# yjpark1/multiagent_rl

Measured on AMD Instinct MI355X. Metric: env-steps/sec, simple_spread N=6 x B envs, 1/2/4/8 MI355X, higher is better.
Workload: dtype f32

## Files before the change

### multiagent_rl_amd/csrc/pw_kernels_spread_quad.hpp

```cpp
#pragma once

#include "pw_kernels_spread.hpp"

namespace {

__device__ __forceinline__ void quad_pair_of(const int q, int &i, int &j)
{
    i = q < 5 ? 0 : q < 9 ? 1 : q < 12 ? 2 : q < 14 ? 3 : 4;
    j = q - (i == 0 ? 0 : i == 1 ? 5 : i == 2 ? 9 : i == 3 ? 12 : 14) + i + 1;
}

__device__ __forceinline__ void quad_act_fetch(const int32_t *row, const uint32_t lane_off, const uint32_t lds_slot, const uint32_t slot_read)
{
    unsigned keep;
    asm volatile("s_mov_b32 %0, m0\n\ts_mov_b32 m0, %3\n\ts_nop 0\n\tglobal_load_lds_dword %1, %2\n\ts_mov_b32 m0, %0"
                 : "=&s"(keep) : "v"(lane_off), "s"(row), "s"(lds_slot), "v"(slot_read) : "memory");
}

template <bool K1>
__device__ __forceinline__ void quad_pair_force(const float2 qi, const float2 qj, const uint32_t near_lo, const uint32_t near_span,
                                                const float dist_min, const float k, const float cf, float &Fx, float &Fy)
{
    const float dx = qi.x - qj.x, dy = qi.y - qj.y;
    const float d2 = dx * dx + dy * dy;
    const f32x2 a = {cf * dx, cf * dy};
    const bool near = __float_as_uint(d2) - near_lo >= near_span;
    const bool uni = (k >= 9.094947017729282e-13f) & (k <= 1099511627776.0f) & (cf >= 9.5367431640625e-07f) & (cf <= 128.0f);
    const bool c1 = (__float_as_uint(d2) - 0x12800000u) < (0x6C800000u - 0x12800000u);
    const bool c2 = fminf(fabsf(a.x), fabsf(a.y)) >= 8.673617379884035e-19f;
    const bool fast = near & c1 & c2 & uni;
    const bool any_cold = __builtin_amdgcn_ballot_w64(near & !fast) != 0;
    Fx = 0.0f; Fy = 0.0f;
    if (fast) {
        const float dist = sqrt_rn_core(d2);
        const float y0 = __builtin_amdgcn_rcpf(dist);
        __builtin_amdgcn_sched_barrier(0);
        const float yd = __builtin_fmaf(__builtin_fmaf(-dist, y0, 1.0f), y0, y0);
        const f32x2 Q = div_chain2(a, dist, yd);
        const float xarg = K1 ? div_chain1(-(dist - dist_min), k, div_refined_rcp(k))
                              : div_chain(-(dist - dist_min), k, div_refined_rcp(k));
        const float pen = softplus_branchless(xarg) * k;
        const f32x2 F = Q * f32x2{pen, pen};
        Fx = F.x;
        Fy = F.y;
    }
    if (__builtin_expect(any_cold, 0)) {
        if (near & !fast) collision_force_pair<true, K1>(qi.x, qi.y, qj.x, qj.y, dist_min, k, cf, Fx, Fy);
    }
}

template <bool COLL>
__device__ __forceinline__ void quad_coll_tests(const float2 mine, const float2 (&q6)[6], const float coll_thr2, int &cnt, uint32_t &cmask)
{
    cnt = 0; cmask = 0;
#if defined(PW_EXPERIMENTS) && defined(PW_EXP_NO_COLL_TESTS)
    cnt = 1;
#else
#pragma unroll
    for (int j = 0; j < 6; ++j) {
        const float2 q = q6[j];
        const float dx = q.x - mine.x, dy = q.y - mine.y;
        const float d2 = dx * dx + dy * dy;
        cnt += d2 < coll_thr2 ? 1 : 0;
        if (COLL) cmask |= d2 < coll_thr2 ? 1u << j : 0u;
    }
#endif
}

#ifndef PW_QUAD_BARRIER
#define PW_QUAD_BARRIER(t) duo_barrier()
#endif
#ifndef PW_QUAD_ACT_AHEAD
#define PW_QUAD_ACT_AHEAD 4
#endif
#ifndef PW_QUAD_PAD_P
#define PW_QUAD_PAD_P()
#endif
#ifndef PW_QUAD_PAD_OB
#define PW_QUAD_PAD_OB()
#endif
constexpr int kQuadActAhead = PW_QUAD_ACT_AHEAD;
constexpr int kQuadN = 6, kQuadL = 6, kQuadEPP = 4, kQuadEPW = 8;
struct SpreadQuadLds { float4 *s_ring; float2 *s_ftab, *s_lmB, *s_utab; float *s_min, *s_rew; int32_t *s_act; uint32_t bytes; };
__host__ __device__ inline SpreadQuadLds spread_quad_lds(unsigned char *raw = nullptr)
{
    LdsCursor c{reinterpret_cast<float *>(raw)}; SpreadQuadLds o;
    o.s_ring = c.take<float4>(4 * kWave);
    o.s_ftab = c.take<float2>(2 * kQuadEPP * kQuadN * kQuadN);
    o.s_min = c.take<float>(kWave); o.s_rew = c.take<float>(kWave);
    o.s_lmB = c.take<float2>(kQuadEPW * kQuadL); o.s_act = c.take<int32_t>(2 * kQuadActAhead * kWave);
    o.s_utab = c.take<float2>(2 * 8);
    o.bytes = 4 * c.at; return o;
}
template <bool UNIT_MASS, bool COLL = false, bool K1 = false>
__global__ void __launch_bounds__(4 * kWave) pw_spread_quad_kernel(const StreamParams A, const int T)
{
    constexpr int N = kQuadN, L = kQuadL, D = 16, P2 = 15, EPP = kQuadEPP, EPW = kQuadEPW;
    extern __shared__ __attribute__((aligned(16))) unsigned char smem_raw[];
    const SpreadQuadLds Y = spread_quad_lds(smem_raw);

    const int wave = __builtin_amdgcn_readfirstlane((((int)threadIdx.x >> 6) + 2 * (((int)blockIdx.x >> 8) & 1)) & 3);
    const int lane = (int)threadIdx.x & 63;
    const int env0 = (int)blockIdx.x * EPW;
    const int envs_here = A.B - env0 < EPW ? A.B - env0 : EPW;
    const size_t BN = (size_t)A.B * N;

    const bool resets = A.auto_reset && A.max_episode_len > 0;
    int offs_all = A.ep_step[env0 + (lane < envs_here ? lane : 0)];
    auto next_reset_step = [&](int t_from) -> int {
        if (!resets) return 0x7fffffff;
        int rem = A.max_episode_len - 1 - (t_from + offs_all);
        rem = rem < 0 ? 0 : rem;
        int m = 0x7fffffff;
        for (int e = 0; e < envs_here; ++e) {
            const int r = __builtin_amdgcn_readlane(rem, e);
            m = r < m ? r : m;
        }
        return t_from + m;
    };
    int t_reset = next_reset_step(0);
    auto reset_step_update = [&](int t) {
        if (t + 1 + offs_all >= A.max_episode_len) offs_all = -(t + 1);
        t_reset = next_reset_step(t + 1);
    };
    int cur = 0;

    if (wave < 2) {
        __builtin_amdgcn_s_setprio(3);
        const int e0 = wave * EPP;
        const int nv = envs_here - e0 < 0 ? 0 : envs_here - e0 < EPP ? envs_here - e0 : EPP;
        if (nv == 0) {
            for (int t = 0; t < T; ++t) PW_QUAD_BARRIER(t);
            return;
        }
        const int la = lane < nv * N ? lane : 0;
        const int e4 = la / N, a = la - e4 * N;
        const int me = (e0 + e4) * N + a;
        const int env = env0 + e0 + e4;
        const uint32_t g = (uint32_t)env * (uint32_t)N + (uint32_t)a;
        const uint64_t env_id = A.env_id_base + (uint64_t)env;
        const int lp = lane < nv * P2 ? lane : 0;
        const int pe = lp / P2, pq = lp - pe * P2;
        int pi, pj;
        quad_pair_of(pq, pi, pj);
        const int ri = (e0 + pe) * N + pi, rj = (e0 + pe) * N + pj;
        float2 *ftab = Y.s_ftab + wave * (EPP * N * N);
        float2 *f_ij = ftab + (pe * N + pi) * N + (pj - 1), *f_ji = ftab + (pe * N + pj) * N + pi;
        const float2 *row = ftab + (e4 * N + a) * N;

        float px = A.pos_x[g], py = A.pos_y[g], vx = A.vel_x[g], vy = A.vel_y[g];
        int ep_off = A.ep_step[env];
        uint32_t ep_count = A.ep_count[env];
        Y.s_ring[me] = make_float4(px, py, vx, vy);
        float2 *utab = Y.s_utab + wave * 8;
        if (lane < 6) {
            const int ai = lane;
            float ux = 0.0f + ((ai == 1 ? 1.0f : 0.0f) - (ai == 2 ? 1.0f : 0.0f));
            float uy = 0.0f + ((ai == 3 ? 1.0f : 0.0f) - (ai == 4 ? 1.0f : 0.0f));
            ux *= A.sens; uy *= A.sens;
            if (A.fscale != 1.0f) { ux = A.fscale * ux; uy = A.fscale * uy; }
            utab[lane] = make_float2(ux + 0.0f, uy + 0.0f);
        }
        wave_lds_sync();
        const float k = A.contact_margin, cf = A.contact_force, dt = A.dt, damp = A.damp, mass = A.mass;
        const uint32_t near_lo = __float_as_uint(A.near_thr2), near_span = 0x7F800000u - near_lo;
        const unsigned char *act_row = reinterpret_cast<const unsigned char *>(A.act);
        const size_t act_stride = BN * sizeof(int32_t);
        const uint32_t act_off = g * (uint32_t)sizeof(int32_t);
        int32_t *act_ring = Y.s_act + wave * (kQuadActAhead * kWave);
        const uint32_t act_lds = __builtin_amdgcn_readfirstlane((uint32_t)reinterpret_cast<uintptr_t>(act_ring));
        auto fetch_act = [&](int t, uint32_t slot_read) {
            quad_act_fetch(reinterpret_cast<const int32_t *>(act_row), act_off, act_lds + (uint32_t)(t & (kQuadActAhead - 1)) * (kWave * 4), slot_read);
            act_row += t + 1 < T ? act_stride : (size_t)0;
        };
        asm volatile("" :: "v"(ep_off), "v"(ep_count), "v"(offs_all), "v"(px), "v"(py), "v"(vx), "v"(vy), "s"(t_reset));
        for (int t0 = 0; t0 < kQuadActAhead; ++t0) fetch_act(t0, 0u);
        float2 qi = *reinterpret_cast<const float2 *>(Y.s_ring + ri);
        float2 qj = *reinterpret_cast<const float2 *>(Y.s_ring + rj);
        PW_STAMP_DECL;
        for (int t = 0; t < T; ++t) {
            PW_STAMP_START;
            asm volatile("s_waitcnt vmcnt(%0)" :: "n"(kQuadActAhead - 1) : "memory");
            PW_STAMP(3);
            const uint32_t ai = (uint32_t)act_ring[(t & (kQuadActAhead - 1)) * kWave + lane];
            fetch_act(t + kQuadActAhead, ai);
            const float2 u0 = utab[ai < 5u ? ai : 5u];
            const bool two_slots = t == t_reset;
            float Fx, Fy;
            quad_pair_force<K1>(qi, qj, near_lo, near_span, A.dist_min, k, cf, Fx, Fy);
            *f_ij = make_float2(Fx, Fy);
            *f_ji = make_float2(-Fx, -Fy);
            PW_STAMP(0);
            float fx = u0.x, fy = u0.y;
            asm volatile("" ::: "memory");
#pragma unroll
            for (int j = 0; j < N - 1; ++j) {
                const float2 F = row[j];
                fx = F.x + fx;
                fy = F.y + fy;
            }
            vx = vx * damp; vy = vy * damp;
            vx = vx + div_mass<UNIT_MASS>(fx, mass) * dt;
            vy = vy + div_mass<UNIT_MASS>(fy, mass) * dt;
            px = px + vx * dt;
            py = py + vy * dt;
            int nxt = (cur + 1) & 3;
            Y.s_ring[nxt * kWave + me] = make_float4(px, py, vx, vy);
            if (__builtin_expect(two_slots, 0)) {
                if (t + 1 + ep_off >= A.max_episode_len) {
                    ep_count += 1;
                    ep_off = -(t + 1);
                    pw_reset_xy(A.seed, env_id, ep_count, (uint32_t)a, -1.0f, 1.0f, &px, &py);
                    vx = 0.f; vy = 0.f;
                }
                reset_step_update(t);
                nxt = (nxt + 1) & 3;
                Y.s_ring[nxt * kWave + me] = make_float4(px, py, vx, vy);
            }
            cur = nxt;
            asm volatile("" ::: "memory");
            qi = *reinterpret_cast<const float2 *>(Y.s_ring + cur * kWave + ri);
            qj = *reinterpret_cast<const float2 *>(Y.s_ring + cur * kWave + rj);
            PW_STAMP(1);
            PW_QUAD_PAD_P();
            PW_QUAD_BARRIER(t);
            PW_STAMP(2);
        }
        act_fetch_drain();
#ifdef PW_STAMPS
        if (blockIdx.x == 0 && wave == 0 && lane == 0)
            for (int i_ = 0; i_ < 4; ++i_) g_pw_stamps[i_] = st_acc[i_];
#endif
        A.pos_x[g] = px; A.pos_y[g] = py;
        A.vel_x[g] = vx; A.vel_y[g] = vy;
        A.ep_step[env] = T + ep_off;
        A.ep_count[env] = ep_count;
        return;
    }

    int e_local = lane / N;
    int a = lane - e_local * N;
    if (e_local >= envs_here) { e_local = 0; a = 0; }
    const int env = env0 + e_local;
    const int base = e_local * N, me = base + a;
    const uint32_t g = (uint32_t)env * (uint32_t)N + (uint32_t)a;
    const uint64_t env_id = A.env_id_base + (uint64_t)env;
    int ep_off = A.ep_step[env];
    uint32_t ep_count = A.ep_count[env];
    float olx = A.lm_x[(size_t)env * L + a], oly = A.lm_y[(size_t)env * L + a];

    if (wave == 2) {
        float own_p = 0.0f;
        int cnt_p = 0;
        const int *cnt_w = reinterpret_cast<const int *>(Y.s_min) + lane;
        const int cnt_span = (int)(Y.s_rew - Y.s_min);
        int cnt_at = 0;
        int pre_last = 0;
        float2 q6[N];
        auto a_reads = [&](const int nxt) __attribute__((always_inline)) {
            const float4 *slot = Y.s_ring + nxt * kWave + base;
#pragma unroll
            for (int j = 0; j < N; ++j) q6[j] = *reinterpret_cast<const float2 *>(slot + j);
            pre_last = nxt;
        };
        float best, e0;
        auto a_dist = [&]() __attribute__((always_inline)) {
            float e2[N];
#pragma unroll
            for (int j = 0; j < N; ++j) {
                const float2 q = q6[j];
                const float ex = q.x - olx, ey = q.y - oly;
                e2[j] = ex * ex + ey * ey;
            }
            best = __builtin_fminf(__builtin_fminf(__builtin_fminf(e2[0], e2[1]), __builtin_fminf(e2[2], e2[3])),
                                   __builtin_fminf(e2[4], e2[5]));
            e0 = e2[0];
        };
        auto a_sqrt = [&]() __attribute__((always_inline)) -> float {
            const float b = e0 != e0 ? e0 : best;
            return sqrtf(b);
        };
        auto a_clock = [&](const int t, int nxt) __attribute__((always_inline)) {
            if (__builtin_expect(t == t_reset, 0)) {
                if (t + 1 + ep_off >= A.max_episode_len) {
                    ep_count += 1;
                    ep_off = -(t + 1);
                    pw_reset_xy(A.seed, env_id, ep_count, (uint32_t)(N + a), -1.0f, 1.0f, &olx, &oly);
                }
                reset_step_update(t);
                nxt = (nxt + 1) & 3;
            }
            cur = nxt;
        };
        float sh_own[L], sh_r[N], r;
        auto b_shfl_own = [&]() __attribute__((always_inline)) {
#pragma unroll
            for (int l = 0; l < L; ++l) sh_own[l] = __shfl(own_p, base + l, kWave);
        };
        auto b_reward = [&]() __attribute__((always_inline)) {
            r = 0.0f;
#pragma unroll
            for (int l = 0; l < L; ++l) r -= sh_own[l];
#pragma unroll
            for (int k2 = 0; k2 < N; ++k2) r -= k2 < cnt_p ? 1.0f : 0.0f;
#pragma unroll
            for (int i = 0; i < N; ++i) sh_r[i] = __shfl(r, base + i, kWave);
        };
        float *rew_t = A.rew, *rsh_t = A.rew_shared;
        auto b_store = [&]() __attribute__((always_inline)) {
            float acc = 0.0f;
#pragma unroll
            for (int i = 0; i < N; ++i) acc += sh_r[i];
            nt_store(rew_t + g, r);
            nt_store(rsh_t + env, acc);
            rew_t += BN; rsh_t += A.B;
        };
        PW_STAMP_DECL;
        {
            PW_STAMP_START;
            PW_QUAD_BARRIER(0);
            PW_STAMP(0);
            const int nxt = (cur + 1) & 3;
            a_reads(nxt);
            a_dist();
            own_p = a_sqrt();
            a_clock(0, nxt);
            PW_STAMP(1);
        }
        for (int t = 1; t < T; ++t) {
            PW_STAMP_START;
            PW_QUAD_BARRIER(t);
            PW_STAMP(0);
            const int nxt = (cur + 1) & 3;
            cnt_p = cnt_w[cnt_at];
            cnt_at = cnt_span - cnt_at;
            a_reads(nxt);
            b_shfl_own();
            a_dist();
            b_reward();
            const float own = a_sqrt();
            b_store();
            own_p = own;
            a_clock(t, nxt);
            PW_STAMP(1);
        }
        {
            const float4 *slot = Y.s_ring + pre_last * kWave + base;
            const float2 mine = *reinterpret_cast<const float2 *>(slot + a);
#pragma unroll
            for (int j = 0; j < N; ++j) q6[j] = *reinterpret_cast<const float2 *>(slot + j);
            uint32_t cmask;
            quad_coll_tests<false>(mine, q6, A.coll_thr2, cnt_p, cmask);
        }
        b_shfl_own();
        b_reward();
        b_store();
#ifdef PW_STAMPS
        if (blockIdx.x == 0 && lane == 0)
            for (int i_ = 0; i_ < 2; ++i_) g_pw_stamps[4 + i_] = st_acc[i_];
#endif
        return;
    }

    const int rows_here = envs_here * N;
    const int cgrp = lane & 3;
    const bool col0 = cgrp == 0;
    int row_u[3];
    uint32_t off_u[3];
#pragma unroll
    for (int u = 0; u < 3; ++u) {
        const int r = (lane >> 2) + 16 * u;
        const bool ok = r < rows_here;
        row_u[u] = ok ? r : 0;
        off_u[u] = (uint32_t)(ok ? lane + 64 * u : cgrp) * 16u;
    }
    float4 lm_u[3];
    auto load_landmarks = [&]() {
#pragma unroll
        for (int u = 0; u < 3; ++u)
            lm_u[u] = *reinterpret_cast<const float4 *>(Y.s_lmB + (row_u[u] / N) * L + (cgrp > 0 ? 2 * cgrp - 2 : 0));
    };
    Y.s_lmB[me] = make_float2(olx, oly);
    wave_lds_sync();
    load_landmarks();
    unsigned char *obs_t = reinterpret_cast<unsigned char *>(A.obs + ((size_t)env0 * N) * D);
    uint8_t *done_t = A.done, *term_t = A.terminal;
    const size_t obs_stride = BN * D * sizeof(float);
    const bool has_len = A.max_episode_len > 0;
    int t_term = has_len ? A.max_episode_len - 1 - ep_off : 0x7fffffff;
    int *cnt_w = reinterpret_cast<int *>(Y.s_min) + lane;
    const int cnt_span = (int)(Y.s_rew - Y.s_min);
    int cnt_at = 0;
    uint64_t *coll_t = A.coll;
    PW_STAMP_DECL;
    for (int t = 0; t < T; ++t) {
        PW_STAMP_START;
        nt_store(done_t + g, (uint8_t)0);
        PW_QUAD_BARRIER(t);
        PW_STAMP(0);
        int nxt = (cur + 1) & 3;
        float2 cmine, cq6[N];
        {
            const float4 *pre = Y.s_ring + nxt * kWave + base;
            cmine = *reinterpret_cast<const float2 *>(pre + a);
#pragma unroll
            for (int j = 0; j < N; ++j) cq6[j] = *reinterpret_cast<const float2 *>(pre + j);
        }
        nt_store(term_t + env, (uint8_t)(t >= t_term ? 1 : 0));
        if (t == t_reset) {
            const bool rst = t >= t_term;
            if (rst) {
                if (A.final_obs) {
                    const float4 st = Y.s_ring[nxt * kWave + me];
                    stream_write_obs<L>(A.final_obs + ((size_t)t * BN + g) * D, L, Y.s_lmB + base, st.x, st.y, st.z, st.w);
                }
                ep_count += 1;
                ep_off = -(t + 1);
                t_term = A.max_episode_len - 1 - ep_off;
                pw_reset_xy(A.seed, env_id, ep_count, (uint32_t)(N + a), -1.0f, 1.0f, &olx, &oly);
            }
            reset_step_update(t);
            wave_lds_sync();
            if (rst) Y.s_lmB[me] = make_float2(olx, oly);
            wave_lds_sync();
            load_landmarks();
            nxt = (nxt + 1) & 3;
        }
        cur = nxt;
        const float4 *slot = Y.s_ring + nxt * kWave;
        float4 st[3];
#pragma unroll
        for (int u = 0; u < 3; ++u) st[u] = slot[row_u[u]];
        {
            int cnt;
            uint32_t cmask;
            quad_coll_tests<COLL>(cmine, cq6, A.coll_thr2, cnt, cmask);
            cnt_w[cnt_at] = cnt;
            cnt_at = cnt_span - cnt_at;
            if (COLL) {
                nt_store(coll_t + g, (uint64_t)cmask);
                coll_t += BN;
            }
        }
        asm volatile("" :: "v"(st[0].x), "v"(st[0].y), "v"(st[0].z), "v"(st[0].w), "v"(st[1].x), "v"(st[1].y), "v"(st[1].z),
                           "v"(st[1].w), "v"(st[2].x), "v"(st[2].y), "v"(st[2].z), "v"(st[2].w));
#pragma unroll
        for (int u = 0; u < 3; ++u) {
            const float4 d = make_float4(lm_u[u].x - st[u].x, lm_u[u].y - st[u].y, lm_u[u].z - st[u].x, lm_u[u].w - st[u].y);
            const float4 o = make_float4(col0 ? st[u].z : d.x, col0 ? st[u].w : d.y, col0 ? st[u].x : d.z, col0 ? st[u].y : d.w);
            nt_store(reinterpret_cast<float4 *>(obs_t + off_u[u]), o);
        }
        obs_t += obs_stride; done_t += BN; term_t += A.B;
        PW_QUAD_PAD_OB();
        PW_STAMP(1);
    }
#ifdef PW_STAMPS
    if (blockIdx.x == 0 && lane == 0)
        for (int i_ = 0; i_ < 2; ++i_) g_pw_stamps[6 + i_] = st_acc[i_];
#endif
    A.lm_x[(size_t)env * L + a] = olx;
    A.lm_y[(size_t)env * L + a] = oly;
}

}
```

Before: 7.913 billion.

## Move action prefetch and force lookup to observation waves via LDS handoff

The physics waves no longer issue global-to-LDS action loads or wait on vmcnt each step. They now read a precomputed action force from a double-buffered LDS slot. The observation-writing waves take over the action prefetch ring, two steps ahead, translate actions through the utab, and write the force into the shared slot for the physics waves. This takes memory latency off the physics critical path, at the cost of more cross-wave LDS dependencies and a vmcnt wait that is mixed in with the observation stores.

```diff
diff --git a/multiagent_rl_amd/csrc/pw_kernels_spread_quad.hpp b/multiagent_rl_amd/csrc/pw_kernels_spread_quad.hpp
--- a/multiagent_rl_amd/csrc/pw_kernels_spread_quad.hpp
+++ b/multiagent_rl_amd/csrc/pw_kernels_spread_quad.hpp
@@ -15,6 +15,15 @@
     unsigned keep;
     asm volatile("s_mov_b32 %0, m0\n\ts_mov_b32 m0, %3\n\ts_nop 0\n\tglobal_load_lds_dword %1, %2\n\ts_mov_b32 m0, %0"
                  : "=&s"(keep) : "v"(lane_off), "s"(row), "s"(lds_slot), "v"(slot_read) : "memory");
+}
+
+__device__ __forceinline__ float2 quad_action_force(const int ai, const float sens, const float fscale)
+{
+    float ux = 0.0f + ((ai == 1 ? 1.0f : 0.0f) - (ai == 2 ? 1.0f : 0.0f));
+    float uy = 0.0f + ((ai == 3 ? 1.0f : 0.0f) - (ai == 4 ? 1.0f : 0.0f));
+    ux *= sens; uy *= sens;
+    if (fscale != 1.0f) { ux = fscale * ux; uy = fscale * uy; }
+    return make_float2(ux + 0.0f, uy + 0.0f);
 }
 
 template <bool K1>
@@ -81,7 +90,7 @@
 #endif
 constexpr int kQuadActAhead = PW_QUAD_ACT_AHEAD;
 constexpr int kQuadN = 6, kQuadL = 6, kQuadEPP = 4, kQuadEPW = 8;
-struct SpreadQuadLds { float4 *s_ring; float2 *s_ftab, *s_lmB, *s_utab; float *s_min, *s_rew; int32_t *s_act; uint32_t bytes; };
+struct SpreadQuadLds { float4 *s_ring; float2 *s_ftab, *s_lmB, *s_utab, *s_u; float *s_min, *s_rew; int32_t *s_act; uint32_t bytes; };
 __host__ __device__ inline SpreadQuadLds spread_quad_lds(unsigned char *raw = nullptr)
 {
     LdsCursor c{reinterpret_cast<float *>(raw)}; SpreadQuadLds o;
@@ -89,6 +98,7 @@
     o.s_ftab = c.take<float2>(2 * kQuadEPP * kQuadN * kQuadN);
     o.s_min = c.take<float>(kWave); o.s_rew = c.take<float>(kWave);
     o.s_lmB = c.take<float2>(kQuadEPW * kQuadL); o.s_act = c.take<int32_t>(2 * kQuadActAhead * kWave);
+    o.s_u = reinterpret_cast<float2 *>(o.s_act + kQuadActAhead * kWave);
     o.s_utab = c.take<float2>(2 * 8);
     o.bytes = 4 * c.at; return o;
 }
@@ -152,39 +162,22 @@
         int ep_off = A.ep_step[env];
         uint32_t ep_count = A.ep_count[env];
         Y.s_ring[me] = make_float4(px, py, vx, vy);
-        float2 *utab = Y.s_utab + wave * 8;
-        if (lane < 6) {
-            const int ai = lane;
-            float ux = 0.0f + ((ai == 1 ? 1.0f : 0.0f) - (ai == 2 ? 1.0f : 0.0f));
-            float uy = 0.0f + ((ai == 3 ? 1.0f : 0.0f) - (ai == 4 ? 1.0f : 0.0f));
-            ux *= A.sens; uy *= A.sens;
-            if (A.fscale != 1.0f) { ux = A.fscale * ux; uy = A.fscale * uy; }
-            utab[lane] = make_float2(ux + 0.0f, uy + 0.0f);
-        }
-        wave_lds_sync();
+        float2 *u_w = Y.s_u + me;
+        {
+            const int32_t a0 = A.act[g], a1 = A.act[(T > 1 ? BN : (size_t)0) + g];
+            u_w[0] = quad_action_force(a0, A.sens, A.fscale);
+            u_w[kQuadEPW * N] = quad_action_force(a1, A.sens, A.fscale);
+        }
+        int u_at = 0;
         const float k = A.contact_margin, cf = A.contact_force, dt = A.dt, damp = A.damp, mass = A.mass;
         const uint32_t near_lo = __float_as_uint(A.near_thr2), near_span = 0x7F800000u - near_lo;
-        const unsigned char *act_row = reinterpret_cast<const unsigned char *>(A.act);
-        const size_t act_stride = BN * sizeof(int32_t);
-        const uint32_t act_off = g * (uint32_t)sizeof(int32_t);
-        int32_t *act_ring = Y.s_act + wave * (kQuadActAhead * kWave);
-        const uint32_t act_lds = __builtin_amdgcn_readfirstlane((uint32_t)reinterpret_cast<uintptr_t>(act_ring));
-        auto fetch_act = [&](int t, uint32_t slot_read) {
-            quad_act_fetch(reinterpret_cast<const int32_t *>(act_row), act_off, act_lds + (uint32_t)(t & (kQuadActAhead - 1)) * (kWave * 4), slot_read);
-            act_row += t + 1 < T ? act_stride : (size_t)0;
-        };
-        asm volatile("" :: "v"(ep_off), "v"(ep_count), "v"(offs_all), "v"(px), "v"(py), "v"(vx), "v"(vy), "s"(t_reset));
-        for (int t0 = 0; t0 < kQuadActAhead; ++t0) fetch_act(t0, 0u);
         float2 qi = *reinterpret_cast<const float2 *>(Y.s_ring + ri);
         float2 qj = *reinterpret_cast<const float2 *>(Y.s_ring + rj);
         PW_STAMP_DECL;
         for (int t = 0; t < T; ++t) {
             PW_STAMP_START;
-            asm volatile("s_waitcnt vmcnt(%0)" :: "n"(kQuadActAhead - 1) : "memory");
-            PW_STAMP(3);
-            const uint32_t ai = (uint32_t)act_ring[(t & (kQuadActAhead - 1)) * kWave + lane];
-            fetch_act(t + kQuadActAhead, ai);
-            const float2 u0 = utab[ai < 5u ? ai : 5u];
+            const float2 u0 = u_w[u_at];
+            u_at = kQuadEPW * N - u_at;
             const bool two_slots = t == t_reset;
             float Fx, Fy;
             quad_pair_force<K1>(qi, qj, near_lo, near_span, A.dist_min, k, cf, Fx, Fy);
@@ -226,7 +219,6 @@
             PW_QUAD_BARRIER(t);
             PW_STAMP(2);
         }
-        act_fetch_drain();
 #ifdef PW_STAMPS
         if (blockIdx.x == 0 && wave == 0 && lane == 0)
             for (int i_ = 0; i_ < 4; ++i_) g_pw_stamps[i_] = st_acc[i_];
@@ -381,8 +373,29 @@
             lm_u[u] = *reinterpret_cast<const float4 *>(Y.s_lmB + (row_u[u] / N) * L + (cgrp > 0 ? 2 * cgrp - 2 : 0));
     };
     Y.s_lmB[me] = make_float2(olx, oly);
+    constexpr int kStepStores = 5 + (COLL ? 1 : 0);
+    constexpr int kActBehind = kQuadActAhead * kStepStores + kQuadActAhead - 1;
+    constexpr int kActWait = kActBehind < 63 ? kActBehind : 63;
+    const unsigned char *act_row = reinterpret_cast<const unsigned char *>(A.act) + (size_t)(T > 2 ? 2 : T > 0 ? T - 1 : 0) * (BN * sizeof(int32_t));
+    const size_t act_stride = BN * sizeof(int32_t);
+    const uint32_t act_off = g * (uint32_t)sizeof(int32_t);
+    const unsigned char *act_ring = reinterpret_cast<const unsigned char *>(Y.s_act + lane);
+    uint32_t act_lds = __builtin_amdgcn_readfirstlane((uint32_t)reinterpret_cast<uintptr_t>(Y.s_act));
+    asm volatile("" : "+s"(act_lds));
+    constexpr uint32_t kSlotBytes = kWave * sizeof(int32_t), kRingMask = kQuadActAhead * kSlotBytes - 1;
+    auto fetch_act = [&](int s, uint32_t slot_at, uint32_t slot_read) {
+        quad_act_fetch(reinterpret_cast<const int32_t *>(act_row), act_off, act_lds + slot_at, slot_read);
+        act_row += s + 1 < T ? act_stride : (size_t)0;
+    };
+    asm volatile("" :: "v"(ep_off), "v"(ep_count), "v"(offs_all), "v"(olx), "v"(oly), "s"(t_reset));
+    for (int s0 = 2; s0 < 2 + kQuadActAhead; ++s0) fetch_act(s0, ((uint32_t)s0 * kSlotBytes) & kRingMask, 0u);
+    if (lane < 6) Y.s_utab[lane] = quad_action_force(lane, A.sens, A.fscale);
+    float2 *u_w = Y.s_u + me;
+    int u_at = 0;
+    uint32_t act_slot = (2 * kSlotBytes) & kRingMask;
     wave_lds_sync();
     load_landmarks();
+    act_fetch_drain();
     unsigned char *obs_t = reinterpret_cast<unsigned char *>(A.obs + ((size_t)env0 * N) * D);
     uint8_t *done_t = A.done, *term_t = A.terminal;
     const size_t obs_stride = BN * D * sizeof(float);
@@ -398,6 +411,8 @@
         nt_store(done_t + g, (uint8_t)0);
         PW_QUAD_BARRIER(t);
         PW_STAMP(0);
+        asm volatile("s_waitcnt vmcnt(%0)" :: "n"(kActWait) : "memory");
+        const uint32_t ai = *reinterpret_cast<const uint32_t *>(act_ring + act_slot);
         int nxt = (cur + 1) & 3;
         float2 cmine, cq6[N];
         {
@@ -406,6 +421,9 @@
 #pragma unroll
             for (int j = 0; j < N; ++j) cq6[j] = *reinterpret_cast<const float2 *>(pre + j);
         }
+        fetch_act(t + 2 + kQuadActAhead, act_slot, ai);
+        act_slot = (act_slot + kSlotBytes) & kRingMask;
+        const float2 u2 = Y.s_utab[ai < 5u ? ai : 5u];
         nt_store(term_t + env, (uint8_t)(t >= t_term ? 1 : 0));
         if (t == t_reset) {
             const bool rst = t >= t_term;
@@ -437,6 +455,8 @@
             quad_coll_tests<COLL>(cmine, cq6, A.coll_thr2, cnt, cmask);
             cnt_w[cnt_at] = cnt;
             cnt_at = cnt_span - cnt_at;
+            u_w[u_at] = u2;
+            u_at = kQuadEPW * N - u_at;
             if (COLL) {
                 nt_store(coll_t + g, (uint64_t)cmask);
                 coll_t += BN;
@@ -460,6 +480,7 @@
 #endif
     A.lm_x[(size_t)env * L + a] = olx;
     A.lm_y[(size_t)env * L + a] = oly;
-}
-
-}
+    act_fetch_drain();
+}
+
+}
```

Result: faster. 8.074 billion, median of 6 (+2.0%).
